# stratosphere/rdfind

Measured on AMD Instinct MI355X. Metric: CIND-discovery triples/sec, higher is better.
Workload: dtype u32

## Files before the change

rdfind_amd/_lib.py:

```python
from __future__ import annotations

import ctypes
import os

import numpy as np

from . import codes

_HERE = os.path.dirname(os.path.abspath(__file__))
LIB_PATH = os.environ.get("RDFIND_HIP_LIB") or os.path.join(_HERE, "librdfind_hip.so")

RDF_CLEAN_IMPLIED = 1
RDF_STRATEGY_ALL_AT_ONCE = 2
RDF_SHARD_LOCAL_SLICE = 4
RDF_USE_ASSOCIATION_RULES = 8

EXPORTED_SYMBOLS = (
    "rdf_ctx_create", "rdf_ctx_destroy", "rdf_last_error", "rdf_version", "rdf_set_triples",
    "rdf_set_triples_device", "rdf_frequent_conditions", "rdf_build_capture_groups", "rdf_discover_cinds",
    "rdf_run", "rdf_cind_count", "rdf_copy_cinds", "rdf_decode_capture", "rdf_binary_key_count",
    "rdf_copy_binary_keys", "rdf_stage_times", "rdf_kernel_times", "rdf_sync",
    "rdf_copy_cinds_range", "rdf_cind_checksum", "rdf_last_stats", "rdf_shard_begin", "rdf_shard_step",
    "rdf_shard_export", "rdf_shard_import", "rdf_set_dictionary", "rdf_format_size", "rdf_format_cinds",
    "rdf_distinct_triples", "rdf_copy_triples", "rdf_parse_ntriples", "rdf_copy_terms",
# ... 4 lines not shown
    "rdf_dictionary_terms", "rdf_copy_result_refs", "rdf_release_scratch", "rdf_set_handover",
    "rdf_copy_result_refs_async", "rdf_handover_wait", "rdf_set_result_form", "rdf_heavy_chunk_count",
    "rdf_copy_result_heavy", "rdf_parse_begin", "rdf_parse_chunk", "rdf_parse_end", "rdf_copy_term_heap",
    "rdf_rewrite_terms", "rdf_condition_histogram", "rdf_join_histogram", "rdf_copy_histogram", "rdf_count_literals",
    "rdf_cind_stats_begin", "rdf_cind_stats_add", "rdf_cind_stats_end", "rdf_cind_histogram", "rdf_copy_top_refs",
    "rdf_select_cinds", "rdf_selected_count", "rdf_copy_selected_decoded", "rdf_format_selected_size",
    "rdf_format_selected", "rdf_find_terms", "rdf_check_cinds", "rdf_copy_check_rows", "rdf_copy_check_examples",
)
RDF_CHK_ABSENT = 0xFFFFFFFE
RDF_CHK_MAX_EXAMPLES = 16
RDF_SEL_ANY = 0xFFFFFFFF
RDF_SEL_MAX_PATTERNS = 256
RDF_SEL_COUNT_ONLY = 1
SEL_CODES = (10, 12, 14, 17, 20, 21, 33, 34, 35)
SEL_ALL_CODES = 0x1FF
RDF_CS_SHAPE, RDF_CS_SUPPORT, RDF_CS_REFS, RDF_CS_INDEGREE = 1, 2, 3, 4
RDF_JH_NO_FIS = 1
RDF_RW_ASCIIFY = 1
RDF_NT_TABS = 1

TEST_SYMBOLS = ("rdf_test_scan", "rdf_test_scan_batch", "rdf_test_radix", "rdf_test_radix_passes",
                "rdf_test_radix_segments", "rdf_test_paths", "rdf_test_rewrite_form", "rdf_test_cind_stats_times",
                "rdf_test_fc_trace", "rdf_test_fc_report", "rdf_test_copy_frequent_unary", "rdf_test_unary_lookup",
                "rdf_test_record_tile", "rdf_test_keep_records", "rdf_test_group_build", "rdf_test_shard_report")
REWRITE_FORMS = {0: None, 1: "lds", 2: "global"}
SCAN_U32_U32, SCAN_U32_U64, SCAN_U64_U64 = range(3)
SCAN_DTYPES = {SCAN_U32_U32: (np.uint32, np.uint32), SCAN_U32_U64: (np.uint32, np.uint64),
               SCAN_U64_U64: (np.uint64, np.uint64)}
RADIX_SORT_BITS, RADIX_SORT_DROP, RADIX_PART_HASHED, RADIX_PART_U32 = range(4)
K1_FORMS = {0: None, 1: "partitioned", 2: "radix", 3: "atomic"}
K2_FORMS = {0: None, 1: "plain", 2: "split", 3: "radix", 4: "atomic"}
K3_FORMS = {0: None, 1: "onepass", 2: "twopass"}

X_DONE, X_ALLREDUCE_SUM_U32, X_ALLREDUCE_SUM_U64, X_ALLREDUCE_MIN_U64, X_ALLGATHERV_U64, X_ALLTOALLV_U64 = range(6)
MAX_RANKS = 64

TIMER_NAMES = ("unary", "binary", "emit", "sort", "support", "groups", "heavymask", "pivot", "light", "esort",
               "hcount", "rules", "hwrite", "class", "cemit")


class FcStats(ctypes.Structure):
    _fields_ = [("min_support", ctypes.c_uint32), ("n_ar_suppressed", ctypes.c_uint32),
                ("n_frequent_unary", ctypes.c_uint64 * 3), ("n_binary_keys", ctypes.c_uint64),
                ("n_frequent_binary", ctypes.c_uint64)]


class ParseStats(ctypes.Structure):
    _fields_ = [("n_triples", ctypes.c_uint64), ("n_terms", ctypes.c_uint64), ("n_lines", ctypes.c_uint64),
                ("n_chunks", ctypes.c_uint64), ("heap_bytes", ctypes.c_uint64), ("table_slots", ctypes.c_uint64),
                ("n_table_growths", ctypes.c_uint64), ("ms", ctypes.c_float)]


class RewriteStats(ctypes.Structure):
    _fields_ = [("n_terms_before", ctypes.c_uint64), ("n_terms_after", ctypes.c_uint64), ("n_changed", ctypes.c_uint64),
                ("heap_bytes", ctypes.c_uint64), ("ms", ctypes.c_float)]
# ... 9 lines not shown

class CindStats(ctypes.Structure):
    _fields_ = [("n_cinds", ctypes.c_uint64), ("n_explicit_raw", ctypes.c_uint64),
                ("n_light_chunks", ctypes.c_uint64), ("n_heavy_chunks", ctypes.c_uint64),
                ("ms_pivot", ctypes.c_float), ("ms_light", ctypes.c_float), ("ms_rules", ctypes.c_float),
                ("ms_heavy", ctypes.c_float), ("n_heavy_candidates", ctypes.c_uint64),
                ("n_class_members", ctypes.c_uint64), ("n_classes", ctypes.c_uint64), ("n_class_cinds", ctypes.c_uint64),
                ("n_light_candidates", ctypes.c_uint64), ("n_light_entries", ctypes.c_uint64)]


class PathReport(ctypes.Structure):
    _fields_ = [("k1_form", ctypes.c_uint32), ("k2_form", ctypes.c_uint32), ("k3_form", ctypes.c_uint32),
                ("dense_on", ctypes.c_uint32), ("light_stage", ctypes.c_uint32), ("light_hiocc", ctypes.c_uint32),
                ("n_dense", ctypes.c_uint64), ("n_dense_eligible", ctypes.c_uint64),
                ("n_dedup_members", ctypes.c_uint64),
                ("n_light_items", ctypes.c_uint64), ("n_packed_octets", ctypes.c_uint64),
                ("n_mseg_chunks", ctypes.c_uint64), ("n_multi_items", ctypes.c_uint64),
                ("n_light_survivors", ctypes.c_uint64),
                ("light_npx", ctypes.c_uint32), ("packed_npx", ctypes.c_uint32), ("light_ordered", ctypes.c_uint32),
                ("light_side", ctypes.c_uint32), ("light_two_pass", ctypes.c_uint32), ("sig_on", ctypes.c_uint32),
                ("piv2_on", ctypes.c_uint32), ("k3_hist", ctypes.c_uint32),
                ("hclassed", ctypes.c_uint32), ("n_class_chunks", ctypes.c_uint64), ("n_emit_tiles", ctypes.c_uint64),
                ("max_class_list", ctypes.c_uint64), ("n_multi_seg_lists", ctypes.c_uint64),
                ("k3_key_items", ctypes.c_uint64), ("k3_suppressed", ctypes.c_uint64)]


class FcReport(ctypes.Structure):
    _fields_ = [("traced", ctypes.c_uint32), ("k1_form", ctypes.c_uint32), ("k1_bits", ctypes.c_uint32),
                ("k2_form", ctypes.c_uint32), ("k2_bits", ctypes.c_uint32), ("k2_sub", ctypes.c_uint32),
                ("k1_buckets", ctypes.c_uint64), ("k1_slices", ctypes.c_uint64), ("k1_multi", ctypes.c_uint64),
                ("k2_buckets", ctypes.c_uint64), ("k2_multi", ctypes.c_uint64), ("k2_spill", ctypes.c_uint64)]


class ShardReport(ctypes.Structure):
    _fields_ = ([("rank", ctypes.c_uint32), ("nranks", ctypes.c_uint32)]
                + [(k, ctypes.c_uint64) for k in (
                    "holder_survivors", "routed_words", "reports_sent", "verify_sent", "reports_received",
                    "verify_received", "verify_kept", "owner_reports", "owner_kept", "unary_own", "binary_own",
                    "unary_gathered", "n_classes", "n_class_members", "n_class_items", "n_list_entries", "hot_entries",
                    "heavy_base", "heavy_columns")]
                + [("have_max_verify", ctypes.c_uint32), ("max_verify_per_dep", ctypes.c_uint64)])


class ResultLayout(ctypes.Structure):
    _fields_ = [(k, ctypes.c_uint64) for k in ("n_cinds", "n_refs", "n_runs", "n_lists", "n_list_refs", "n_members",
                                                "n_captures")]

# ... 154 lines not shown
        "rdf_shard_step": (i32, [P, ctypes.POINTER(Exchange)]),
        "rdf_shard_export": (i32, [P, P]),
        "rdf_shard_import": (i32, [P, P, u64]),
        "rdf_test_scan": (i32, [P, ctypes.c_int, P, u64, u32, u32, ctypes.c_int, ctypes.c_int, P, ctypes.POINTER(u64),
                                ctypes.POINTER(u32)]),
        "rdf_test_scan_batch": (i32, [P, ctypes.c_int, P, u64, u32, P, ctypes.POINTER(u32)]),
        "rdf_test_radix": (i32, [P, ctypes.c_int, P, u64, ctypes.c_int, ctypes.c_int, u64, P, ctypes.POINTER(u64),
                                 ctypes.POINTER(u32)]),
        "rdf_test_radix_passes": (ctypes.c_int, [ctypes.c_int]),
        "rdf_test_radix_segments": (i32, [P, P, u64, P, u64, P, u32, ctypes.c_int, ctypes.c_int, ctypes.c_int32, u32, u32,
                                          P, ctypes.POINTER(u64), ctypes.POINTER(u32)]),
        "rdf_test_paths": (i32, [P, ctypes.POINTER(PathReport)]),
        "rdf_test_rewrite_form": (i32, [P, ctypes.POINTER(u32)]),
        "rdf_test_cind_stats_times": (i32, [P, ctypes.POINTER(ctypes.c_float)]),
        "rdf_test_fc_trace": (i32, [P, ctypes.c_int]),
        "rdf_test_fc_report": (i32, [P, ctypes.POINTER(FcReport)]),
        "rdf_test_shard_report": (i32, [P, ctypes.POINTER(ShardReport)]),
        "rdf_test_copy_frequent_unary": (i32, [P, P, u64, ctypes.POINTER(u64), ctypes.POINTER(u64)]),
        "rdf_test_unary_lookup": (i32, [P, P, u64, P, P, ctypes.POINTER(u32)]),
        "rdf_test_record_tile": (ctypes.c_int, []),
        "rdf_test_keep_records": (i32, [P, P, u64, ctypes.c_int, u64, u32, P, ctypes.POINTER(u64), ctypes.POINTER(u32), P, P,
                                        P, ctypes.POINTER(u32)]),
        "rdf_test_group_build": (i32, [P, P, u64, u32, u64, u32, ctypes.POINTER(u64), P, P, P, ctypes.POINTER(u32)]),
    }
    for name, (res, args) in sig.items():
        fn = getattr(lib, name, None) if name in TEST_SYMBOLS else getattr(lib, name)
        if fn is None:
            continue
        fn.restype = res
        fn.argtypes = args
    _lib = lib
    return lib


class PinnedBuffer:

    def __init__(self, count: int, dtype):
        self.lib = load()
        self.nbytes = max(int(count), 1) * np.dtype(dtype).itemsize
        self.ptr = self.lib.rdf_host_alloc(self.nbytes)
        if not self.ptr:
            raise RdfError(f"rdf_host_alloc({self.nbytes}) failed")
        self.array = np.ctypeslib.as_array((ctypes.c_uint8 * self.nbytes).from_address(self.ptr)).view(dtype)

    def __del__(self):
        if getattr(self, "ptr", None):
# ... 443 lines not shown
        dk, fk = np.empty(max(a.shape[0], 1), np.uint64), np.empty(max(a.shape[0], 1), np.uint64)
        doff = np.empty(ncap + 1, np.uint64)
        jf, ncomp, ok = ctypes.c_uint64(), ctypes.c_uint32(), ctypes.c_uint32()
        rc = self._test_fn("rdf_test_keep_records")(
            self.ptr, a.ctypes.data, a.shape[0], joinbits, ncap, ms, sup.ctypes.data, ctypes.byref(jf), ctypes.byref(ncomp),
            dk.ctypes.data, fk.ctypes.data, doff.ctypes.data, ctypes.byref(ok))
        self.test_canaries_ok = bool(ok.value)
        self._check(rc, "rdf_test_keep_records")
        return sup, dk[: jf.value], fk[: jf.value], doff[: ncomp.value + 1], bool(ok.value)

    def test_group_build(self, fk, num_values: int, rbase=0, gbase=0):
        a = np.ascontiguousarray(fk, dtype=np.uint64)
        goff = np.empty(a.shape[0] + 1, np.uint64)
        gcap = np.empty(max(a.shape[0], 1), np.uint32)
        gmap = np.empty(num_values, np.uint32)
        g, ok = ctypes.c_uint64(), ctypes.c_uint32()
        rc = self._test_fn("rdf_test_group_build")(
            self.ptr, a.ctypes.data, a.shape[0], num_values, rbase, gbase, ctypes.byref(g), goff.ctypes.data,
            gcap.ctypes.data, gmap.ctypes.data, ctypes.byref(ok))
        self.test_canaries_ok = bool(ok.value)
        self._check(rc, "rdf_test_group_build")
        return goff[: g.value + 1], gcap[: a.shape[0]], gmap, bool(ok.value)

    def test_paths(self) -> dict:
        r = PathReport()
        self._check(self._test_fn("rdf_test_paths")(self.ptr, ctypes.byref(r)), "rdf_test_paths")
        d = _struct_dict(r)
        d["k1_form"], d["k2_form"], d["k3_form"] = K1_FORMS[r.k1_form], K2_FORMS[r.k2_form], K3_FORMS[r.k3_form]
        for name in ("dense_on", "light_stage", "light_hiocc", "light_ordered", "light_side", "light_two_pass", "sig_on",
                     "piv2_on", "k3_hist", "hclassed"):
            d[name] = bool(d[name])
        return d

    def test_shard_report(self) -> dict:
        r = ShardReport()
        self._check(self._test_fn("rdf_test_shard_report")(self.ptr, ctypes.byref(r)), "rdf_test_shard_report")
        d = _struct_dict(r)
        if not d.pop("have_max_verify"):
            d["max_verify_per_dep"] = None
        return d

    def test_fc_trace(self, on: bool = True):
        self._check(self._test_fn("rdf_test_fc_trace")(self.ptr, int(on)), "rdf_test_fc_trace")

    def test_fc_report(self) -> dict:
        r = FcReport()
        self._check(self._test_fn("rdf_test_fc_report")(self.ptr, ctypes.byref(r)), "rdf_test_fc_report")
        d = _struct_dict(r)
        d["k1_form"], d["k2_form"], d["traced"] = K1_FORMS[r.k1_form], K2_FORMS[r.k2_form], bool(r.traced)
        return d

# ... 260 lines not shown
```

rdfind_amd/csrc/primitives.hip:

```cpp
#include <cstdint>
#include <cstdlib>
#include <type_traits>

#include "primitives.hpp"
#include "radix_host.hpp"
#include "switches.hpp"

namespace rdf {


typedef unsigned int u32x4_t __attribute__((ext_vector_type(4)));
typedef unsigned long long u64x2_t __attribute__((ext_vector_type(2)));

template <typename T>
__device__ inline T block_exclusive_scan(T v, T* lds_wave, T* total) {
    const int lane = lane_id();
    const int wave = threadIdx.x / RDF_WAVE;
    T incl = v;
#pragma unroll
    for (int off = 1; off < RDF_WAVE; off <<= 1) {
        T t = __shfl_up(incl, off, RDF_WAVE);
        if (lane >= off) incl += t;
    }
    if (lane == RDF_WAVE - 1) lds_wave[wave] = incl;
// ... 908 lines not shown
        shift += w;
    }
    return hipGetLastError();
}

hipError_t radix_partition_u32(Workspace& ws, u32*& keys, u32*& tmp, u64 n, int lo, int hi, hipStream_t st) {
    if (n < 2 || hi <= lo) return hipSuccess;
    if (n >= (1ull << 32) || hi > 32) return hipErrorInvalidValue;
    const u32 tiles = (u32)((n + RS_TILE - 1) / RS_TILE);
    const int bits = hi - lo, passes = (bits + 7) / 8;
    u32* hist = (u32*)ws.scratch(((u64)hist_stride(tiles) << 8) * sizeof(u32), 1);
    if (!hist) return hipErrorOutOfMemory;
    int shift = lo;
    for (int p = 0; p < passes; ++p) {
        const int w = bits / passes + (p < bits % passes ? 1 : 0);
        hipError_t e = radix_pass<8, false, u32>(ws, keys, tmp, n, shift, w, hist, tiles, st);
        if (e != hipSuccess) return e;
        std::swap(keys, tmp);
        shift += w;
    }
    return hipGetLastError();
}

}
```

rdfind_amd/csrc/primitives.hpp:

```cpp
#pragma once
#include "common.hpp"

namespace rdf {

struct DevBuf {
    void* p = nullptr;
    size_t cap = 0;
    hipError_t ensure(size_t bytes) {
        if (bytes <= cap && p) return hipSuccess;
        if (p) {
            hipError_t e = hipFree(p);
            if (e != hipSuccess) return e;
            p = nullptr;
            cap = 0;
        }
        size_t want = bytes < 256 ? 256 : bytes;
        hipError_t e = hipMalloc(&p, want);
        if (e != hipSuccess) {
            p = nullptr;
            (void)hipGetLastError();
            return e;
        }
        cap = want;
        return hipSuccess;
// ... 52 lines not shown
hipError_t exclusive_scan_u32_u64_batch(Workspace& ws, const u32* const* in, u64* const* out, int k, u64 n,
                                        hipStream_t st);
hipError_t exclusive_scan_u64(Workspace& ws, const u64* in, u64* out, u64 n, u64* d_total, hipStream_t st);
hipError_t exclusive_scan_u32(Workspace& ws, const u32* in, u32* out, u64 n, u32* d_total, hipStream_t st);

hipError_t radix_sort_u64(Workspace& ws, u64*& keys, u64*& tmp, u64 n, int bits, hipStream_t st);
#ifndef RDF_RS_MAX_BITS
#define RDF_RS_MAX_BITS 9
#endif
static constexpr int RS_MAX_BITS = RDF_RS_MAX_BITS;
static_assert(RS_MAX_BITS >= 8 && RS_MAX_BITS <= 10, "digit kernels exist for 8, 9 and 10 bits");
hipError_t radix_sort_u64_drop(Workspace& ws, u64*& keys, u64*& tmp, u64 n, int bits, u32* d_kept, u64* n_out,
                               hipStream_t st);
hipError_t radix_sort_u64_bits(Workspace& ws, u64*& keys, u64*& tmp, u64 n, int lo, int hi, hipStream_t st);
int radix_first_width(int bits);
u32 radix_seg_stride(u32 columns);
u32* radix_seg_hist(Workspace& ws, u32 columns, int w);
hipError_t radix_seg_first_pass(Workspace& ws, const u64* src, u64 src_n, u64* dst, u64 n_out, const u64* base, u64 stride,
                                const u64* cnt, u32 columns, int w, u32* hist, u32* d_overflow, hipStream_t st);
hipError_t radix_sort_u64_rest(Workspace& ws, u64*& keys, u64*& tmp, u64 n, int w0, int bits, hipStream_t st);
int radix_sort_passes(int bits);
hipError_t radix_partition_hashed(Workspace& ws, u64*& keys, u64*& tmp, u64 n, int bits, u64 hmask, hipStream_t st);
hipError_t radix_partition_u32(Workspace& ws, u32*& keys, u32*& tmp, u64 n, int lo, int hi, hipStream_t st);

}
```

rdfind_amd/csrc/rdfind_hip.hip:

```cpp
#include <algorithm>
#include <cstdio>
#include <cstring>
#include <cstdlib>
#include <string>
#include <chrono>
#include <vector>
#include <utility>
#include <initializer_list>
#include <unordered_map>

#include "../../include/rdfind_hip.h"
#include "test_abi.h"
#include "primitives.hpp"
#include "radix_host.hpp"
#include "kernels.inl"
#include "switches.hpp"

using namespace rdf;

#define RDF_VERSION "rdfind_amd 0.1 (gfx950)"

#define RDF_CTX_BUFFERS(B) \
     \
    B(INPUT, scal) \
// ... 222 lines not shown
    bool light_hiocc = false;
    u64 light_wmean = 0;
    bool pivx_on = false;
    int pivx_kept = 0;
    int light_npx = 0;
    u32* dbits_p = nullptr;
    hipStream_t side = nullptr;
    hipEvent_t ev_fork = nullptr, ev_join = nullptr;
    hipStream_t hstream = nullptr;
    hipEvent_t hv_ev = nullptr;
    uint32_t *hv_refs = nullptr, *hv_capid = nullptr, *hv_sup = nullptr, *hv_rundep = nullptr;
    uint64_t* hv_runoff = nullptr;
    u64 hv_refs_cap = 0, hv_cap_cap = 0, hv_runs_cap = 0;
    u64 hv_runs_n = ~0ull;
    u64 hv_refs_n = ~0ull;
    bool hv_caps_done = false;
    bool hv_pending = false;
    hipEvent_t hv_done = nullptr;
    bool hv_gpu_wait = false;
    bool dense_on = false;
    u64 dwords = 0, n_dense = 0;
    bool dense_flagged = false;
    u64 n_dense_eligible = 0;
    u32 path_k1 = 0, path_k2 = 0, path_k3 = 0;
    bool fc_trace = false;
    rdf_test_fc_report_t fcrep = {};
    rdf_test_shard_report_t shrep = {};
    bool shrep_done = false;
    u64 shrep_vC = ~0ull;
    bool k3_hist = false;
    u64 k3_key_items = 0, k3_suppressed = 0;
    struct LightPaths {
        u64 items = 0, packed_octets = 0, mseg_chunks = 0;
        int light_npx = 0, packed_npx = 0;
        bool ordered = false, side = false, two_pass = false;
    } lpaths;
    bool sig_on = false;
    bool sig_packed = false;
    bool piv2_on = false;
    bool piv2_packed = true;
    u64 n_class_members = 0, n_classes = 0, n_class_out = 0;
    bool class_pending = false;
    u64 pend_NT = 0, pend_base = 0, n_lists = 0, n_list_refs = 0, n_runs_explicit = 0;
    u32 result_form = 0;
    u64 res_K = 0, res_nx = 0, res_wh = 0, res_h0 = 0;
    bool res_bits = false;
    bool heavy_pending = false;
// ... 1626 lines not shown
    return (u64)(4 + frac) << (msb - 2);
}

static rdf_status parse_projection(rdf_ctx* c, const char* projection, int* proj) {
    const char* pr = projection ? projection : "spo";
    int m = 0;
    for (const char* q = pr; *q; ++q) {
        if (*q == 's') m |= 1;
        else if (*q == 'p') m |= 2;
        else if (*q == 'o') m |= 4;
        else return fail(c, RDF_ERR_ARG, std::string("invalid projection attribute in '") + pr + "'");
    }
    *proj = m;
    return RDF_OK;
}


static rdf_status g_record_bits(rdf_ctx* c) {
    c->spare_groups = false;
    c->jr_keep = false;
    c->dense_on = false;
    c->n_dense = c->n_dense_eligible = c->n_dedup_members = 0;
    c->path_k3 = 0;
    c->k3_hist = false;
    c->k3_key_items = c->k3_suppressed = 0;
    const u32 V = c->V ? c->V : 1;
    const u64 ncap = 2ull * c->U + c->B;
    const int capbits = bits_for(ncap ? ncap - 1 : 0);
    const int joinbits = bits_for(V - 1);
    if (capbits + joinbits > 64) return fail(c, RDF_ERR_LIMIT, "join+capture bits exceed 64");
    if (6ull * V + c->B >= (1ull << 32)) return fail(c, RDF_ERR_LIMIT, "capture id space exceeds 2^32");
    c->capbits = capbits;
    c->joinbits = joinbits;
    c->ncap = ncap;
    return RDF_OK;
}

static JoinSel shard_sel(const rdf_ctx* c) {
    JoinSel js{c->rank, c->nranks, 0u, JOIN_ALL_HI};
    if (c->nranks > 1 && c->hot_n) {
        js.hot = c->hot.as<u64>();
        js.hmask = c->hot_mask;
    }
    return js;
}

// ... 227 lines not shown
    hipLaunchKernelGGL(k_support_flags, dim3(grid_for(ncap, RDF_BLOCK, kGrid)), dim3(RDF_BLOCK), 0, st,
                       c->support.as<u32>(), ncap, c->ms, c->flags.as<u32>());
    HIP_TRY(c, exclusive_scan_u32(c->ws, c->flags.as<u32>(), c->fidx.as<u32>(), ncap, c->fidx.as<u32>() + ncap, st));
    u32 C = 0, Cu = 0;
    {
        u64 v[2];
        TRY(read_multi(c, {{c->fidx.as<u32>() + ncap, 4}, {c->fidx.as<u32>() + 2ull * c->U, 4}}, v));
        C = (u32)v[0];
        Cu = (u32)v[1];
    }
    c->C = C;
    c->Cu = Cu;
    ENSURE(c, fcap, std::max<u64>(C, 1) * 4);
    ENSURE(c, info, std::max<u64>(C, 1) * sizeof(CapInfo));
    hipLaunchKernelGGL(k_compact_captures, dim3(grid_for(ncap, RDF_BLOCK, kGrid)), dim3(RDF_BLOCK), 0, st,
                       c->support.as<u32>(), c->fidx.as<u32>(), ncap, c->ms, c->fcap.as<u32>(), c->info.as<CapInfo>());
    ENSURE(c, fext, std::max<u64>(C, 1) * 4);
    if (C)
        hipLaunchKernelGGL(k_external_ids, dim3(grid_for(C, RDF_BLOCK, kGrid)), dim3(RDF_BLOCK), 0, st, c->fcap.as<u32>(), C,
                           2u * c->U, V, c->fval.as<u32>(), c->Us, c->Up, c->fext.as<u32>());
    return RDF_OK;
}

static rdf_status g_group_heads(rdf_ctx* c, u64 Jr, u32* Gout) {
    hipStream_t st = c->stream;
    const unsigned nt = rec_tiles(Jr);
    ENSURE(c, tile_heads, std::max<u64>(nt, 1) * 4);
    ENSURE(c, tile_gbase, (nt + 1ull) * 4);
    if (nt) hipLaunchKernelGGL(k_group_flags, dim3(nt), dim3(RDF_BLOCK), 0, st, c->fk.as<u64>(), Jr, c->tile_heads.as<u32>());
    HIP_TRY(c, exclusive_scan_u32(c->ws, c->tile_heads.as<u32>(), c->tile_gbase.as<u32>(), nt, c->tile_gbase.as<u32>() + nt, st));
    return read_u32(c, c->tile_gbase.as<u32>() + nt, Gout);
}

static rdf_status g_compact_groups(rdf_ctx* c, const u32* local_sup) {
    hipStream_t st = c->stream;
    const u32 V = c->V ? c->V : 1;
    const u64 ncap = c->ncap, J = c->J;
    const int joinbits = c->joinbits;
    u64* keys = c->rec_sorted;
    tbegin(c, RDF_T_SUPPORT);
    TRY(g_compact_captures(c));
    const u32 C = c->C;
    ENSURE(c, skip, (ncap + 1) * 4);
    if (ncap)
        hipLaunchKernelGGL(k_skip_counts, dim3(grid_for(ncap, RDF_BLOCK, kGrid)), dim3(RDF_BLOCK), 0, st,
                           local_sup ? local_sup : c->support.as<u32>(), c->support.as<u32>(), ncap, c->ms, c->flags.as<u32>());
    HIP_TRY(c, exclusive_scan_u32(c->ws, c->flags.as<u32>(), c->skip.as<u32>(), ncap, c->skip.as<u32>() + ncap, st));
    const unsigned nt = rec_tiles(J);
    u64 fs[2];
    TRY(read_multi(c, {{c->tile_base.as<u32>() + nt, 4}, {c->skip.as<u32>() + ncap, 4}}, fs));
    const u64 Jf = fs[0] - fs[1];
    c->Jf = Jf;
    u64* dk = keys == c->rec.as<u64>() ? c->rec_tmp.as<u64>() : c->rec.as<u64>();
    ENSURE(c, fk, std::max<u64>(Jf, 1) * 8);
    ENSURE(c, fk_tmp, std::max<u64>(Jf, 1) * 8);
    if (nt)
        hipLaunchKernelGGL(k_keep_scatter, dim3(nt), dim3(RDF_BLOCK), 0, st, keys, J, joinbits, c->tile_base.as<u32>(),
                           c->skip.as<u32>(), c->support.as<u32>(), c->ms, c->fidx.as<u32>(), dk, c->fk.as<u64>());
    tend(c, RDF_T_SUPPORT);
    tbegin(c, RDF_T_GROUPS);
    ENSURE(c, csup, std::max<u64>(C, 1) * 4);
    ENSURE(c, doff, (C + 1ull) * 8);
    ENSURE(c, dgrp, std::max<u64>(Jf, 1) * 4);
    if (C)
        hipLaunchKernelGGL(k_info_support_u32, dim3(grid_for(C, RDF_BLOCK, kGrid)), dim3(RDF_BLOCK), 0, st,
                           c->info.as<CapInfo>(), C, c->csup.as<u32>());
    const u32* nrec = c->csup.as<u32>();
    if (local_sup) {
        ENSURE(c, dcur, std::max<u64>(C, 1) * 4);
        if (C)
            hipLaunchKernelGGL(k_gather_u32, dim3(grid_for(C, RDF_BLOCK, kGrid)), dim3(RDF_BLOCK), 0, st, local_sup,
                               c->fcap.as<u32>(), (u64)C, c->dcur.as<u32>());
        nrec = c->dcur.as<u32>();
    }
    HIP_TRY(c, exclusive_scan_u32_u64(c->ws, nrec, c->doff.as<u64>(), C, c->doff.as<u64>() + C, st));
    if (Jf) {
        u64* tk = c->fk.as<u64>();
        u64* tt = c->fk_tmp.as<u64>();
        HIP_TRY(c, radix_sort_u64_bits(c->ws, tk, tt, Jf, 32, 32 + joinbits, st));
        if (tk != c->fk.as<u64>()) std::swap(c->fk, c->fk_tmp);
    }
    u32 G32 = 0;
    TRY(g_group_heads(c, Jf, &G32));
    const u64 G = G32;
    c->G = G;
    ENSURE(c, goff, (G + 1) * 8);
    ENSURE(c, gcap, std::max<u64>(Jf, 1) * 4 + 16);
    ENSURE(c, gmap, (u64)V * 4);
    if (Jf) {
        hipLaunchKernelGGL(k_group_build, dim3(rec_tiles(Jf)), dim3(RDF_BLOCK), 0, st, c->fk.as<u64>(), Jf,
                           c->tile_gbase.as<u32>(), c->goff.as<u64>(), c->gcap.as<u32>(), c->gmap.as<u32>());
        hipLaunchKernelGGL(k_dgrp, dim3(grid_for(Jf, RDF_BLOCK, kGrid)), dim3(RDF_BLOCK), 0, st, dk, Jf, c->gmap.as<u32>(),
                           c->dgrp.as<u32>());
    }
    c->hscal[14] = Jf;
    HIP_TRY(c, hipMemcpyAsync(c->goff.as<u64>() + G, c->hscal + 14, 8, hipMemcpyHostToDevice, st));
    tend(c, RDF_T_GROUPS);
    return RDF_OK;
}

static rdf_status g_range_keep_plan(rdf_ctx* c) {
    const std::vector<rdf_ctx::JoinRange>& ranges = c->jranges;
    c->jr_keep = false;
    if (!c->sw.range_keep || ranges.empty() || ranges.size() > EMIT_MAX_RANGES) return RDF_OK;
    u64 total = 0;
    c->jr_seg.assign(ranges.size() + 1, 0);
    c->jr_J.assign(ranges.size(), 0);
    for (size_t k = 0; k < ranges.size(); ++k) {
        c->jr_seg[k] = total;
        total += ranges[k].recs;
    }
    c->jr_seg[ranges.size()] = total;
// ... 228 lines not shown
        if (ncap)
            hipLaunchKernelGGL(k_skip_counts, dim3(grid_for(ncap, RDF_BLOCK, kGrid)), dim3(RDF_BLOCK), 0, st, c->rsup.as<u32>(),
                               c->support.as<u32>(), ncap, c->ms, c->flags.as<u32>());
        HIP_TRY(c, exclusive_scan_u32(c->ws, c->flags.as<u32>(), c->skip.as<u32>(), ncap, c->skip.as<u32>() + ncap, st));
        const unsigned nt = rec_tiles(J);
        u64 fs[2];
        TRY(read_multi(c, {{c->tile_base.as<u32>() + nt, 4}, {c->skip.as<u32>() + ncap, 4}}, fs));
        const u64 Jr = fs[0] - fs[1];
        u64* dk = keys == c->rec.as<u64>() ? c->rec_tmp.as<u64>() : c->rec.as<u64>();
        ENSURE(c, fk, std::max<u64>(Jr, 1) * 8);
        ENSURE(c, fk_tmp, std::max<u64>(Jr, 1) * 8);
        if (nt)
            hipLaunchKernelGGL(k_keep_scatter, dim3(nt), dim3(RDF_BLOCK), 0, st, keys, J, joinbits, c->tile_base.as<u32>(),
                               c->skip.as<u32>(), c->support.as<u32>(), c->ms, c->fidx.as<u32>(), dk, c->fk.as<u64>());
        tend(c, RDF_T_SUPPORT);
        tbegin(c, RDF_T_GROUPS);
        if (Jr) {
            u64* tk = c->fk.as<u64>();
            u64* tt = c->fk_tmp.as<u64>();
            HIP_TRY(c, radix_sort_u64_bits(c->ws, tk, tt, Jr, 32, 32 + joinbits, st));
            if (tk != c->fk.as<u64>()) std::swap(c->fk, c->fk_tmp);
        }
        u32 Gr = 0;
        TRY(g_group_heads(c, Jr, &Gr));
        if (G0 + Gr > Gmax || Jf0 + Jr > Jf) return fail(c, RDF_ERR_LIMIT, "join ranges disagree on the kept records");
        if (Jr) {
            hipLaunchKernelGGL(k_group_build_at, dim3(rec_tiles(Jr)), dim3(RDF_BLOCK), 0, st, c->fk.as<u64>(), Jr,
                               c->tile_gbase.as<u32>(), Jf0, (u32)G0, c->goff.as<u64>(), c->gcap.as<u32>(), c->gmap.as<u32>());
            hipLaunchKernelGGL(k_key_offsets, dim3(grid_for(C + 1ull, RDF_BLOCK, kGrid)), dim3(RDF_BLOCK), 0, st, dk, Jr, C,
                               c->offp.as<u64>());
            hipLaunchKernelGGL(k_dgrp_range, dim3(grid_for(Jr, RDF_BLOCK, kGrid)), dim3(RDF_BLOCK), 0, st, dk, Jr,
                               c->offp.as<u64>(), c->doff.as<u64>(), c->dcur.as<u32>(), c->gmap.as<u32>(), c->dgrp.as<u32>());
            if (C)
                hipLaunchKernelGGL(k_dcur_add, dim3(grid_for(C, RDF_BLOCK, kGrid)), dim3(RDF_BLOCK), 0, st, c->offp.as<u64>(), C,
                                   c->dcur.as<u32>());
        }
        tend(c, RDF_T_GROUPS);
        Jf0 += Jr;
        G0 += Gr;
    }
    if (Jf0 != Jf) return fail(c, RDF_ERR_LIMIT, "join ranges disagree on the kept records");
    c->G = G0;
    c->J = Jtot;
    c->J_emit = J_emit;
    c->hscal[14] = Jf;
    HIP_TRY(c, hipMemcpyAsync(c->goff.as<u64>() + G0, c->hscal + 14, 8, hipMemcpyHostToDevice, st));
    HIP_TRY(c, hipStreamSynchronize(st));
// ... 4020 lines not shown
```

rdfind_amd/csrc/switches.hpp:

```cpp
#pragma once
#include <algorithm>
#include <cstdio>
#include <cstdlib>
#include <cstring>
#include <string>

#include "common.hpp"

namespace rdf {

template <typename T>
struct Opt {
    bool set = false;
    T v{};
};
static inline Opt<int> opt_int(const char* v) { return {true, atoi(v)}; }
static inline Opt<u64> opt_u64(const char* v) { return {true, strtoull(v, nullptr, 10)}; }
static inline Opt<std::string> opt_str(const char* v) { return {true, v}; }
static inline bool is_set(const char*) { return true; }
static inline u64 positive_or(const char* v, u64 dflt) { return atoll(v) > 0 ? (u64)atoll(v) : dflt; }
struct RankPhase {
    int rank = -1, phase = -1;
};
static inline RankPhase rank_phase(const char* v) {
// ... 12 lines not shown
       "0: K2 never groups its records by hash prefix (no k_b2_emit / k_b2_split)") \
    SW(b2_radix_min, u64, B2_RADIX_MIN, "RDFIND_B2_RADIX_MIN", strtoull(v, nullptr, 10), TEST, \
       "3n from which K2 groups compact records with the radix passes") \
     \
    SW(nt_dict_slots, u64, 1ull << 16, "RDFIND_NT_DICT_SLOTS", positive_or(v, s.nt_dict_slots), TEST, \
       "=<pow2>: initial slots of the chunked parse's persistent term table (small: tiny inputs rebuild it several times)") \
    SW(nt_fp_bits, int, 32, "RDFIND_NT_FP_BITS", std::max(0, std::min(atoi(v), 32)), TEST, \
       "=<0..32>: fingerprint bits the chunked parse compares before the bytes (0: every occupied slot is byte-compared)") \
     \
    SW(heavy_min, u64, 64, "RDFIND_HEAVY_MIN", positive_or(v, s.heavy_min), TEST, \
       "minimum heavy-group size (a power of two; smaller groups are cheaper by binary search than as bit columns)") \
    SW(group_range_records, u64, 0, "RDFIND_GROUP_RANGE", positive_or(v, s.group_range_records), TEST, \
       "build the capture groups in join ranges of at most that many K3 records (0: only from 2^32 / 9 triples, automatic size)") \
    SW(range_keep, bool, true, "RDFIND_RANGE_KEEP", atoi(v) != 0, TEST, \
       "0: pass 2 of a range build always re-emits (as when pass 1's records do not fit)") \
    SW(emit_onepass, bool, true, "RDFIND_EMIT_ONEPASS", atoi(v) != 0, TEST, \
       "0: K3 as count pass + write pass (as when the record buffers hold fewer than 9 records per triple)") \
    SW(emit_hist, bool, true, "RDFIND_EMIT_HIST", atoi(v) != 0, AB, \
       "0: the one-pass K3 compacts its regions and the record sort counts its first digit itself (no histogram from K3)") \
    SW(emit_keys, bool, true, "RDFIND_EMIT_KEYS", atoi(v) != 0, AB, \
       "0: K3 has no key items: every triple writes the two unary records its frequent binary keys determine") \
    SW(emit_grid, u64, 0, "RDFIND_EMIT_GRID", strtoull(v, nullptr, 10), TEST, \
       "=<blocks>: cap of K3's emission grid (small: a small input's blocks emit regions of several sort sub-tiles)") \
     \
    SW(allow_hclass, bool, true, "RDFIND_HCLASS", strcmp(v, "0") != 0, AB, \
       "=0: binary heavy-only dependents are not emitted from class lists") \
    SW(dense_div, int, -1, "RDFIND_DENSE", atoi(v), AB, \
       "bitmaps for light groups of >= C / <divisor> members on every input (0: none; unset: by input, d_dense_flags)") \
    SW(dense_min, u64, LIGHT_DENSE_MIN, "RDFIND_DENSE_MIN", positive_or(v, s.dense_min), TEST, \
       "absolute minimum size of a dense light group (bitmaps for small groups too)") \
    SW(dense_bytes, u64, DENSE_BYTES, "RDFIND_DENSE_BYTES", (u64)atoll(v), TEST, \
       "cap of the dense bitmaps' bytes (rows past the cap stay member lists)") \
    SW(sig, int, 2, "RDFIND_SIG", atoi(v), AB, \
       "light-group signatures: 0 off, 1 tested by k_light and the packed path, 2 by k_light only") \
    SW(piv2, int, 1, "RDFIND_PIV2", atoi(v), AB, \
       "second pivots: 0 off, 1 checked by k_light and the packed path, 2 by k_light only") \
    SW(pivx, bool, true, "RDFIND_PIVX", atoi(v) != 0, AB, \
       "0: no extra pivots after the second one (there are none without RDFIND_PIV2 either)") \
    SW(pivx_n, Opt<int>, {}, "RDFIND_PIVX_N", opt_int(v), AB, \
       "how many of the computed extra pivots k_light checks (unset: all the variant takes)") \
    SW(pivx_packed, Opt<int>, {}, "RDFIND_PIVX_PACKED", opt_int(v), TEST, \
       "0 / 1: the packed path checks the first extra pivot (unset: on large-group inputs)") \
    SW(stage, Opt<int>, {}, "RDFIND_STAGE", opt_int(v), TEST, \
       "0 / 1: k_light stages light groups in LDS rows (unset: by the weighted mean light group size)") \
    SW(light_hiocc, Opt<int>, {}, "RDFIND_LIGHT_HIOCC", opt_int(v), TEST, \
       "0 / 1: the plain k_light at 6 waves per SIMD (unset: by input; never with the staging variant)") \
// ... 65 lines not shown
```

Before: 1.670 billion.

## Build capture groups from split u32 join/capture pairs instead of u64 records

The one-pass group build now keeps its records as separate u32 join and capture arrays and sorts them with a new key-value u32 radix sort over only the join bits. The group heads, group build and dependent-group kernels get kv variants that read these arrays, and the separate fk/fk_tmp u64 buffers are no longer allocated on this path. The aim is to cut the memory traffic and passes of sorting 64-bit packed records. It adds new kernels and buffer-aliasing logic, and a switch (on by default) keeps the old u64 path available.

```diff
diff --git a/rdfind_amd/_lib.py b/rdfind_amd/_lib.py
--- a/rdfind_amd/_lib.py
+++ b/rdfind_amd/_lib.py
@@ -50,7 +50,8 @@
 TEST_SYMBOLS = ("rdf_test_scan", "rdf_test_scan_batch", "rdf_test_radix", "rdf_test_radix_passes",
                 "rdf_test_radix_segments", "rdf_test_paths", "rdf_test_rewrite_form", "rdf_test_cind_stats_times",
                 "rdf_test_fc_trace", "rdf_test_fc_report", "rdf_test_copy_frequent_unary", "rdf_test_unary_lookup",
-                "rdf_test_record_tile", "rdf_test_keep_records", "rdf_test_group_build", "rdf_test_shard_report")
+                "rdf_test_record_tile", "rdf_test_keep_records", "rdf_test_group_build", "rdf_test_shard_report",
+                "rdf_test_radix_pairs", "rdf_test_group_kv")
 REWRITE_FORMS = {0: None, 1: "lds", 2: "global"}
 SCAN_U32_U32, SCAN_U32_U64, SCAN_U64_U64 = range(3)
 SCAN_DTYPES = {SCAN_U32_U32: (np.uint32, np.uint32), SCAN_U32_U64: (np.uint32, np.uint64),
@@ -59,6 +60,7 @@
 K1_FORMS = {0: None, 1: "partitioned", 2: "radix", 3: "atomic"}
 K2_FORMS = {0: None, 1: "plain", 2: "split", 3: "radix", 4: "atomic"}
 K3_FORMS = {0: None, 1: "onepass", 2: "twopass"}
+GROUP_FORMS = {0: None, 1: "u64", 2: "kv"}
 
 X_DONE, X_ALLREDUCE_SUM_U32, X_ALLREDUCE_SUM_U64, X_ALLREDUCE_MIN_U64, X_ALLGATHERV_U64, X_ALLTOALLV_U64 = range(6)
 MAX_RANKS = 64
@@ -114,7 +116,8 @@
                 ("piv2_on", ctypes.c_uint32), ("k3_hist", ctypes.c_uint32),
                 ("hclassed", ctypes.c_uint32), ("n_class_chunks", ctypes.c_uint64), ("n_emit_tiles", ctypes.c_uint64),
                 ("max_class_list", ctypes.c_uint64), ("n_multi_seg_lists", ctypes.c_uint64),
-                ("k3_key_items", ctypes.c_uint64), ("k3_suppressed", ctypes.c_uint64)]
+                ("k3_key_items", ctypes.c_uint64), ("k3_suppressed", ctypes.c_uint64),
+                ("group_form", ctypes.c_uint32)]
 
 
 class FcReport(ctypes.Structure):
@@ -315,6 +318,9 @@
         "rdf_test_keep_records": (i32, [P, P, u64, ctypes.c_int, u64, u32, P, ctypes.POINTER(u64), ctypes.POINTER(u32), P, P,
                                         P, ctypes.POINTER(u32)]),
         "rdf_test_group_build": (i32, [P, P, u64, u32, u64, u32, ctypes.POINTER(u64), P, P, P, ctypes.POINTER(u32)]),
+        "rdf_test_radix_pairs": (i32, [P, P, P, u64, ctypes.c_int, ctypes.c_int, P, P, ctypes.POINTER(u32)]),
+        "rdf_test_group_kv": (i32, [P, P, u64, ctypes.c_int, u64, u32, u32, P, ctypes.POINTER(u64), ctypes.POINTER(u32), P, P,
+                                    ctypes.POINTER(u64), P, P, P, ctypes.POINTER(u32)]),
     }
     for name, (res, args) in sig.items():
         fn = getattr(lib, name, None) if name in TEST_SYMBOLS else getattr(lib, name)
@@ -804,11 +810,40 @@
         self._check(rc, "rdf_test_group_build")
         return goff[: g.value + 1], gcap[: a.shape[0]], gmap, bool(ok.value)
 
+    def test_radix_pairs(self, keys, vals, lo=0, hi=32):
+        k = np.ascontiguousarray(keys, dtype=np.uint32)
+        v = np.ascontiguousarray(vals, dtype=np.uint32)
+        assert k.shape == v.shape
+        ko, vo = np.empty_like(k), np.empty_like(v)
+        ok = ctypes.c_uint32()
+        rc = self._test_fn("rdf_test_radix_pairs")(self.ptr, k.ctypes.data, v.ctypes.data, k.shape[0], lo, hi,
+                                                   ko.ctypes.data, vo.ctypes.data, ctypes.byref(ok))
+        self.test_canaries_ok = bool(ok.value)
+        self._check(rc, "rdf_test_radix_pairs")
+        return ko, vo, bool(ok.value)
+
+    def test_group_kv(self, keys, joinbits: int, ncap: int, ms: int, num_values: int) -> dict:
+        a = np.ascontiguousarray(keys, dtype=np.uint64)
+        m = max(a.shape[0], 1)
+        sup, doff = np.empty(ncap, np.uint32), np.empty(ncap + 1, np.uint64)
+        dgrp, gcap = np.empty(m, np.uint32), np.empty(m, np.uint32)
+        goff, gmap = np.empty(m + 1, np.uint64), np.empty(num_values, np.uint32)
+        jf, g, ncomp, ok = ctypes.c_uint64(), ctypes.c_uint64(), ctypes.c_uint32(), ctypes.c_uint32()
+        rc = self._test_fn("rdf_test_group_kv")(
+            self.ptr, a.ctypes.data, a.shape[0], joinbits, ncap, ms, num_values, sup.ctypes.data, ctypes.byref(jf),
+            ctypes.byref(ncomp), doff.ctypes.data, dgrp.ctypes.data, ctypes.byref(g), goff.ctypes.data, gcap.ctypes.data,
+            gmap.ctypes.data, ctypes.byref(ok))
+        self.test_canaries_ok = bool(ok.value)
+        self._check(rc, "rdf_test_group_kv")
+        return {"support": sup, "doff": doff[: ncomp.value + 1], "dgrp": dgrp[: jf.value], "goff": goff[: g.value + 1],
+                "gcap": gcap[: jf.value], "gmap": gmap, "G": g.value, "Jf": jf.value, "canaries_ok": bool(ok.value)}
+
     def test_paths(self) -> dict:
         r = PathReport()
         self._check(self._test_fn("rdf_test_paths")(self.ptr, ctypes.byref(r)), "rdf_test_paths")
         d = _struct_dict(r)
         d["k1_form"], d["k2_form"], d["k3_form"] = K1_FORMS[r.k1_form], K2_FORMS[r.k2_form], K3_FORMS[r.k3_form]
+        d["group_form"] = GROUP_FORMS[r.group_form]
         for name in ("dense_on", "light_stage", "light_hiocc", "light_ordered", "light_side", "light_two_pass", "sig_on",
                      "piv2_on", "k3_hist", "hclassed"):
             d[name] = bool(d[name])
diff --git a/rdfind_amd/csrc/primitives.hip b/rdfind_amd/csrc/primitives.hip
--- a/rdfind_amd/csrc/primitives.hip
+++ b/rdfind_amd/csrc/primitives.hip
@@ -954,4 +954,213 @@
     return hipGetLastError();
 }
 
-}
+
+__device__ inline void load_tile_quads(const u32* __restrict__ a, u64 n, u64 tbase, u32 (&k)[RS_ITEMS]) {
+    static_assert(RS_ITEMS % 4 == 0, "a lane loads whole quads");
+#pragma unroll
+    for (int r = 0; r < RS_ITEMS / 4; ++r) {
+        const u64 idx = tbase + 4ull * ((u64)r * RDF_BLOCK + threadIdx.x);
+        if (idx + 3 < n) {
+            const u32x4_t v = *(const u32x4_t*)(a + idx);
+            k[4 * r] = v.x;
+            k[4 * r + 1] = v.y;
+            k[4 * r + 2] = v.z;
+            k[4 * r + 3] = v.w;
+        } else {
+#pragma unroll
+            for (int q = 0; q < 4; ++q) k[4 * r + q] = idx + q < n ? a[idx + q] : 0u;
+        }
+    }
+}
+
+template <int DB>
+__global__ __launch_bounds__(RDF_BLOCK) void k_radix_count_kv(const u32* __restrict__ keys, u64 n, int shift, int w,
+                                                              u32* __restrict__ hist, u32 num_tiles) {
+    constexpr u32 NBIN = 1u << DB;
+    __shared__ u32 wcnt[RDF_WAVES_PER_BLOCK][NBIN];
+    const int lane = lane_id();
+    const int wave = threadIdx.x / RDF_WAVE;
+    const u32 dmask = (1u << w) - 1u;
+    for (u32 i = threadIdx.x; i < RDF_WAVES_PER_BLOCK * NBIN; i += RDF_BLOCK) (&wcnt[0][0])[i] = 0;
+    __syncthreads();
+    const u32 tile = rs_tile();
+    const u64 tbase = (u64)tile * RS_TILE;
+    u32 k[RS_ITEMS];
+    load_tile_quads(keys, n, tbase, k);
+#pragma unroll
+    for (int r = 0; r < RS_ITEMS; ++r) {
+        const bool valid = tbase + 4ull * ((u64)(r / 4) * RDF_BLOCK + threadIdx.x) + (r & 3) < n;
+        const u32 d = (k[r] >> shift) & dmask;
+        const u64 peers = digit_peers<DB>(d, valid);
+        if (valid && ((peers >> lane) >> 1) == 0) wcnt[wave][d] += (u32)__popcll(peers);
+    }
+    __syncthreads();
+    for (u32 b = threadIdx.x; b <= dmask; b += RDF_BLOCK) {
+        u32 sum = 0;
+#pragma unroll
+        for (int ww = 0; ww < RDF_WAVES_PER_BLOCK; ++ww) sum += wcnt[ww][b];
+        hist[(u64)b * num_tiles + tile] = sum;
+    }
+}
+
+template <int DB>
+__global__ __launch_bounds__(RDF_BLOCK) void k_radix_scatter_kv(const u32* __restrict__ keys, const u32* __restrict__ vals,
+                                                                u32* __restrict__ okeys, u32* __restrict__ ovals, u64 n,
+                                                                int shift, int w, const u32* __restrict__ offs,
+                                                                const u32* __restrict__ rowtot, u32 num_tiles) {
+    constexpr u32 NBIN = 1u << DB;
+    constexpr u32 PER = NBIN / RDF_BLOCK;
+    static_assert(NBIN % RDF_BLOCK == 0, "digit bins must be a multiple of the block");
+    __shared__ __align__(16) u32 skeys[RS_TILE];
+    __shared__ __align__(16) u32 svals[RS_TILE];
+    __shared__ u32 wcount[RDF_WAVES_PER_BLOCK][NBIN];
+    __shared__ u32 tstart[NBIN];
+    __shared__ u32 gbase[NBIN];
+    __shared__ u32 lds_wave[RDF_WAVES_PER_BLOCK];
+    const int lane = lane_id();
+    const int wave = threadIdx.x / RDF_WAVE;
+    const u32 nbin = 1u << w, dmask = nbin - 1u;
+    for (u32 i = threadIdx.x; i < RDF_WAVES_PER_BLOCK * NBIN; i += RDF_BLOCK) (&wcount[0][0])[i] = 0;
+    const u32 tile = rs_tile();
+    const u64 tbase = (u64)tile * RS_TILE;
+    const u32 tn = n - tbase < (u64)RS_TILE ? (u32)(n - tbase) : (u32)RS_TILE;
+    {
+        u32 kin[RS_ITEMS], vin[RS_ITEMS];
+        load_tile_quads(keys, n, tbase, kin);
+        load_tile_quads(vals, n, tbase, vin);
+        u32 rt[PER], ro[PER], local = 0;
+#pragma unroll
+        for (u32 q = 0; q < PER; ++q) {
+            const u32 dg = threadIdx.x * PER + q;
+            rt[q] = dg < nbin ? rowtot[dg] : 0u;
+            ro[q] = dg < nbin ? offs[(u64)dg * num_tiles + tile] : 0u;
+            local += rt[q];
+        }
+        u32 total;
+        u32 off = block_exclusive_scan<u32>(local, lds_wave, &total);
+#pragma unroll
+        for (u32 q = 0; q < PER; ++q) {
+            gbase[threadIdx.x * PER + q] = off + ro[q];
+            off += rt[q];
+        }
+#pragma unroll
+        for (int r = 0; r < RS_ITEMS / 4; ++r) {
+            const u32 p = 4u * ((u32)r * RDF_BLOCK + threadIdx.x);
+            *(u32x4_t*)(skeys + p) = u32x4_t{kin[4 * r], kin[4 * r + 1], kin[4 * r + 2], kin[4 * r + 3]};
+            *(u32x4_t*)(svals + p) = u32x4_t{vin[4 * r], vin[4 * r + 1], vin[4 * r + 2], vin[4 * r + 3]};
+        }
+    }
+    __syncthreads();
+    u32 k[RS_ITEMS], v[RS_ITEMS], rank[RS_ITEMS];
+    const u64 lt = lanemask_lt();
+    const u32 wofs = (u32)wave * RS_WAVE_KEYS;
+#pragma unroll
+    for (int r = 0; r < RS_ITEMS; ++r) {
+        k[r] = skeys[wofs + (u32)r * RDF_WAVE + lane];
+        v[r] = svals[wofs + (u32)r * RDF_WAVE + lane];
+    }
+#pragma unroll
+    for (int r = 0; r < RS_ITEMS; ++r) {
+        const bool valid = wofs + (u32)r * RDF_WAVE + lane < tn;
+        const u32 d = (k[r] >> shift) & dmask;
+        const u64 peers = digit_peers<DB>(d, valid);
+        const u32 before = (u32)__popcll(peers & lt);
+        const u32 old = valid ? wcount[wave][d] : 0;
+        if (valid && ((peers >> lane) >> 1) == 0) wcount[wave][d] = old + before + 1;
+        rank[r] = old + before;
+    }
+    __syncthreads();
+    {
+        u32 run[PER], local = 0;
+#pragma unroll
+        for (u32 q = 0; q < PER; ++q) {
+            const u32 dg = threadIdx.x * PER + q;
+            u32 acc = 0;
+#pragma unroll
+            for (int ww = 0; ww < RDF_WAVES_PER_BLOCK; ++ww) {
+                const u32 c = wcount[ww][dg];
+                wcount[ww][dg] = acc;
+                acc += c;
+            }
+            run[q] = acc;
+            local += acc;
+        }
+        u32 total;
+        u32 off = block_exclusive_scan<u32>(local, lds_wave, &total);
+#pragma unroll
+        for (u32 q = 0; q < PER; ++q) {
+            tstart[threadIdx.x * PER + q] = off;
+            off += run[q];
+        }
+    }
+    __syncthreads();
+#pragma unroll
+    for (int r = 0; r < RS_ITEMS; ++r) {
+        if (wofs + (u32)r * RDF_WAVE + lane < tn) {
+            const u32 d = (k[r] >> shift) & dmask;
+            const u32 p = tstart[d] + wcount[wave][d] + rank[r];
+            skeys[p] = k[r];
+            svals[p] = v[r];
+        }
+    }
+    __syncthreads();
+#pragma unroll
+    for (int i = 0; i < RS_ITEMS; ++i) {
+        const u32 p = (u32)i * RDF_BLOCK + threadIdx.x;
+        if (p < tn) {
+            const u32 key = skeys[p];
+            const u32 d = (key >> shift) & dmask;
+            const u64 at = (u64)gbase[d] + (p - tstart[d]);
+            okeys[at] = key;
+            ovals[at] = svals[p];
+        }
+    }
+}
+
+template <int DB>
+static hipError_t radix_pass_kv(Workspace& ws, const u32* keys, const u32* vals, u32* okeys, u32* ovals, u64 n, int shift,
+                                int w, u32* hist, u32 tiles, hipStream_t st) {
+    u32* rowtot = (u32*)ws.scratch(1024 * sizeof(u32), 2);
+    if (!rowtot) return hipErrorOutOfMemory;
+    const u32 rs = hist_stride(tiles);
+    hipLaunchKernelGGL(k_radix_count_kv<DB>, dim3(tiles), dim3(RDF_BLOCK), 0, st, keys, n, shift, w, hist, rs);
+    hipLaunchKernelGGL(k_radix_rowscan, dim3(1u << w), dim3(RS_SCAN_THREADS), 0, st, hist, rs, tiles, rowtot);
+    hipLaunchKernelGGL(k_radix_scatter_kv<DB>, dim3(tiles), dim3(RDF_BLOCK), 0, st, keys, vals, okeys, ovals, n, shift, w, hist,
+                       rowtot, rs);
+    return hipGetLastError();
+}
+
+hipError_t radix_sort_pairs_u32(Workspace& ws, const u32* keys_in, const u32* vals_in, u32* keys_out, u32* vals_out,
+                                u32* keys_tmp, u32* vals_tmp, u64 n, int lo, int hi, hipStream_t st) {
+    if (n == 0) return hipSuccess;
+    if (n >= (1ull << 32) || lo < 0 || hi > 32) return hipErrorInvalidValue;
+    for (const u32* a : {keys_in, vals_in, (const u32*)keys_out, (const u32*)vals_out, (const u32*)keys_tmp, (const u32*)vals_tmp})
+        if (!a || ((uintptr_t)a & 15u)) return hipErrorInvalidValue;
+    const int bits = hi - lo, dmax = sort_digit_bits(bits);
+    const int passes = n < 2 || bits <= 0 ? 0 : (bits + dmax - 1) / dmax;
+    if (passes == 0) {
+        hipError_t e = hipMemcpyAsync(keys_out, keys_in, n * 4, hipMemcpyDeviceToDevice, st);
+        if (e == hipSuccess) e = hipMemcpyAsync(vals_out, vals_in, n * 4, hipMemcpyDeviceToDevice, st);
+        return e;
+    }
+    const u32 tiles = (u32)((n + RS_TILE - 1) / RS_TILE);
+    u32* hist = (u32*)ws.scratch(((u64)hist_stride(tiles) << dmax) * sizeof(u32), 1);
+    if (!hist) return hipErrorOutOfMemory;
+    const u32 *sk = keys_in, *sv = vals_in;
+    int shift = lo;
+    for (int p = 0; p < passes; ++p) {
+        const int w = bits / passes + (p < bits % passes ? 1 : 0);
+        const bool to_out = ((passes - 1 - p) & 1) == 0;
+        u32 *dk = to_out ? keys_out : keys_tmp, *dv = to_out ? vals_out : vals_tmp;
+        hipError_t e = w <= 8 ? radix_pass_kv<8>(ws, sk, sv, dk, dv, n, shift, w, hist, tiles, st)
+                     : w == 9 ? radix_pass_kv<9>(ws, sk, sv, dk, dv, n, shift, w, hist, tiles, st)
+                              : radix_pass_kv<10>(ws, sk, sv, dk, dv, n, shift, w, hist, tiles, st);
+        if (e != hipSuccess) return e;
+        sk = dk;
+        sv = dv;
+        shift += w;
+    }
+    return hipGetLastError();
+}
+
+}
diff --git a/rdfind_amd/csrc/primitives.hpp b/rdfind_amd/csrc/primitives.hpp
--- a/rdfind_amd/csrc/primitives.hpp
+++ b/rdfind_amd/csrc/primitives.hpp
@@ -98,5 +98,7 @@
 int radix_sort_passes(int bits);
 hipError_t radix_partition_hashed(Workspace& ws, u64*& keys, u64*& tmp, u64 n, int bits, u64 hmask, hipStream_t st);
 hipError_t radix_partition_u32(Workspace& ws, u32*& keys, u32*& tmp, u64 n, int lo, int hi, hipStream_t st);
+hipError_t radix_sort_pairs_u32(Workspace& ws, const u32* keys_in, const u32* vals_in, u32* keys_out, u32* vals_out,
+                                u32* keys_tmp, u32* vals_tmp, u64 n, int lo, int hi, hipStream_t st);
 
 }
diff --git a/rdfind_amd/csrc/rdfind_hip.hip b/rdfind_amd/csrc/rdfind_hip.hip
--- a/rdfind_amd/csrc/rdfind_hip.hip
+++ b/rdfind_amd/csrc/rdfind_hip.hip
@@ -268,7 +268,7 @@
     u64 dwords = 0, n_dense = 0;
     bool dense_flagged = false;
     u64 n_dense_eligible = 0;
-    u32 path_k1 = 0, path_k2 = 0, path_k3 = 0;
+    u32 path_k1 = 0, path_k2 = 0, path_k3 = 0, path_group_kv = 0;
     bool fc_trace = false;
     rdf_test_fc_report_t fcrep = {};
     rdf_test_shard_report_t shrep = {};
@@ -1941,6 +1941,7 @@
     c->dense_on = false;
     c->n_dense = c->n_dense_eligible = c->n_dedup_members = 0;
     c->path_k3 = 0;
+    c->path_group_kv = 0;
     c->k3_hist = false;
     c->k3_key_items = c->k3_suppressed = 0;
     const u32 V = c->V ? c->V : 1;
@@ -2214,12 +2215,13 @@
     return RDF_OK;
 }
 
-static rdf_status g_group_heads(rdf_ctx* c, u64 Jr, u32* Gout) {
+static rdf_status g_group_heads(rdf_ctx* c, u64 Jr, const u32* sj, u32* Gout) {
     hipStream_t st = c->stream;
     const unsigned nt = rec_tiles(Jr);
     ENSURE(c, tile_heads, std::max<u64>(nt, 1) * 4);
     ENSURE(c, tile_gbase, (nt + 1ull) * 4);
-    if (nt) hipLaunchKernelGGL(k_group_flags, dim3(nt), dim3(RDF_BLOCK), 0, st, c->fk.as<u64>(), Jr, c->tile_heads.as<u32>());
+    if (nt && sj) hipLaunchKernelGGL(k_group_flags_kv, dim3(nt), dim3(RDF_BLOCK), 0, st, sj, Jr, c->tile_heads.as<u32>());
+    else if (nt) hipLaunchKernelGGL(k_group_flags, dim3(nt), dim3(RDF_BLOCK), 0, st, c->fk.as<u64>(), Jr, c->tile_heads.as<u32>());
     HIP_TRY(c, exclusive_scan_u32(c->ws, c->tile_heads.as<u32>(), c->tile_gbase.as<u32>(), nt, c->tile_gbase.as<u32>() + nt, st));
     return read_u32(c, c->tile_gbase.as<u32>() + nt, Gout);
 }
@@ -2243,10 +2245,23 @@
     TRY(read_multi(c, {{c->tile_base.as<u32>() + nt, 4}, {c->skip.as<u32>() + ncap, 4}}, fs));
     const u64 Jf = fs[0] - fs[1];
     c->Jf = Jf;
-    u64* dk = keys == c->rec.as<u64>() ? c->rec_tmp.as<u64>() : c->rec.as<u64>();
-    ENSURE(c, fk, std::max<u64>(Jf, 1) * 8);
-    ENSURE(c, fk_tmp, std::max<u64>(Jf, 1) * 8);
-    if (nt)
+    const bool kv = c->sw.group_kv;
+    c->path_group_kv = kv ? RDF_TEST_GROUPS_KV : RDF_TEST_GROUPS_U64;
+    const bool keys_in_rec = keys == c->rec.as<u64>();
+    DevBuf& kept = keys_in_rec ? c->rec_tmp : c->rec;
+    const u64 Jq = (Jf + 3) & ~3ull;
+    if (kv) {
+        TRY(ensure_buf(c, &kept, std::max<u64>(Jq, 4) * 8, "allocating the kept joins and captures"));
+    } else {
+        ENSURE(c, fk, std::max<u64>(Jf, 1) * 8);
+        ENSURE(c, fk_tmp, std::max<u64>(Jf, 1) * 8);
+    }
+    u64* dk = kept.as<u64>();
+    u32 *joins = kept.as<u32>(), *caps = kept.as<u32>() + Jq;
+    if (nt && kv)
+        hipLaunchKernelGGL(k_keep_scatter_kv, dim3(nt), dim3(RDF_BLOCK), 0, st, keys, J, joinbits, c->tile_base.as<u32>(),
+                           c->skip.as<u32>(), c->support.as<u32>(), c->ms, c->fidx.as<u32>(), joins, caps);
+    else if (nt)
         hipLaunchKernelGGL(k_keep_scatter, dim3(nt), dim3(RDF_BLOCK), 0, st, keys, J, joinbits, c->tile_base.as<u32>(),
                            c->skip.as<u32>(), c->support.as<u32>(), c->ms, c->fidx.as<u32>(), dk, c->fk.as<u64>());
     tend(c, RDF_T_SUPPORT);
@@ -2266,20 +2281,31 @@
         nrec = c->dcur.as<u32>();
     }
     HIP_TRY(c, exclusive_scan_u32_u64(c->ws, nrec, c->doff.as<u64>(), C, c->doff.as<u64>() + C, st));
-    if (Jf) {
+    const u32* sj = c->dgrp.as<u32>();
+    ENSURE(c, gcap, std::max<u64>(Jf, 1) * 4 + 16);
+    if (Jf && kv) {
+        DevBuf& spent = keys_in_rec ? c->rec : c->rec_tmp;
+        TRY(ensure_buf(c, &spent, Jq * 8, "allocating the pair sort's scratch"));
+        HIP_TRY(c, radix_sort_pairs_u32(c->ws, joins, caps, c->dgrp.as<u32>(), c->gcap.as<u32>(), spent.as<u32>(),
+                                        spent.as<u32>() + Jq, Jf, 0, joinbits, st));
+    } else if (Jf) {
         u64* tk = c->fk.as<u64>();
         u64* tt = c->fk_tmp.as<u64>();
         HIP_TRY(c, radix_sort_u64_bits(c->ws, tk, tt, Jf, 32, 32 + joinbits, st));
         if (tk != c->fk.as<u64>()) std::swap(c->fk, c->fk_tmp);
     }
     u32 G32 = 0;
-    TRY(g_group_heads(c, Jf, &G32));
+    TRY(g_group_heads(c, Jf, kv ? sj : nullptr, &G32));
     const u64 G = G32;
     c->G = G;
     ENSURE(c, goff, (G + 1) * 8);
-    ENSURE(c, gcap, std::max<u64>(Jf, 1) * 4 + 16);
     ENSURE(c, gmap, (u64)V * 4);
-    if (Jf) {
+    if (Jf && kv) {
+        hipLaunchKernelGGL(k_group_build_kv, dim3(rec_tiles(Jf)), dim3(RDF_BLOCK), 0, st, sj, Jf, c->tile_gbase.as<u32>(),
+                           c->goff.as<u64>(), c->gmap.as<u32>());
+        hipLaunchKernelGGL(k_dgrp_kv, dim3(grid_for(Jf, RDF_BLOCK, kGrid)), dim3(RDF_BLOCK), 0, st, joins, Jf,
+                           c->gmap.as<u32>(), c->dgrp.as<u32>());
+    } else if (Jf) {
         hipLaunchKernelGGL(k_group_build, dim3(rec_tiles(Jf)), dim3(RDF_BLOCK), 0, st, c->fk.as<u64>(), Jf,
                            c->tile_gbase.as<u32>(), c->goff.as<u64>(), c->gcap.as<u32>(), c->gmap.as<u32>());
         hipLaunchKernelGGL(k_dgrp, dim3(grid_for(Jf, RDF_BLOCK, kGrid)), dim3(RDF_BLOCK), 0, st, dk, Jf, c->gmap.as<u32>(),
@@ -2554,7 +2580,7 @@
             if (tk != c->fk.as<u64>()) std::swap(c->fk, c->fk_tmp);
         }
         u32 Gr = 0;
-        TRY(g_group_heads(c, Jr, &Gr));
+        TRY(g_group_heads(c, Jr, nullptr, &Gr));
         if (G0 + Gr > Gmax || Jf0 + Jr > Jf) return fail(c, RDF_ERR_LIMIT, "join ranges disagree on the kept records");
         if (Jr) {
             hipLaunchKernelGGL(k_group_build_at, dim3(rec_tiles(Jr)), dim3(RDF_BLOCK), 0, st, c->fk.as<u64>(), Jr,
diff --git a/rdfind_amd/csrc/switches.hpp b/rdfind_amd/csrc/switches.hpp
--- a/rdfind_amd/csrc/switches.hpp
+++ b/rdfind_amd/csrc/switches.hpp
@@ -58,6 +58,8 @@
        "0: K3 has no key items: every triple writes the two unary records its frequent binary keys determine") \
     SW(emit_grid, u64, 0, "RDFIND_EMIT_GRID", strtoull(v, nullptr, 10), TEST, \
        "=<blocks>: cap of K3's emission grid (small: a small input's blocks emit regions of several sort sub-tiles)") \
+    SW(group_kv, bool, true, "RDFIND_GROUP_KV", atoi(v) != 0, AB, \
+       "0: the one-pass group build keeps and sorts its records as u64 (dk, fk), not as u32 joins and captures") \
      \
     SW(allow_hclass, bool, true, "RDFIND_HCLASS", strcmp(v, "0") != 0, AB, \
        "=0: binary heavy-only dependents are not emitted from class lists") \
```

After: 1.715 billion, median of 6. +2.7%, better.
